# shroglck/open-pi-zero

Measured on AMD Instinct MI355X. Metric: train samples/sec at gbsz 1024 (bf16 fwd+bwd+clip+AdamW), higher is better.
Workload: dtype bf16; 1 GPU; Pi0 bridge training step: 256 img + 20 text + 1 proprio + 4 action tokens; model=pi0 (SigLIP-So400m/14 + Gemma-2B + 0.3B action expert), global_batch=1024, micro_batch=256, grad_accum=4, seq_len=281, parallelism=dp1

## Files before the change

include/pz_abi.h:

```cpp
#ifndef PZ_ABI_H
#define PZ_ABI_H

#include <stdint.h>

#ifdef __cplusplus
extern "C" {
#endif

#define PZ_ABI_VERSION 22

enum {
  PZ_OK = 0,
  PZ_ERR_INVALID_ARG = 1,
  PZ_ERR_LAUNCH = 2,
  PZ_ERR_UNSUPPORTED = 3,
};

enum {
  PZ_EPI_NONE = 0,
  PZ_EPI_GELU = 1,
  PZ_EPI_GEGLU = 2,
  PZ_EPI_SILU = 3,
  PZ_EPI_DGELU = 4,
  PZ_EPI_DSILU = 5,
// ... 47 lines not shown
  float alpha;
  int32_t beta;
} pz_small_gemm_args;
int pz_gemm_small(const pz_small_gemm_args* args, void* stream);

int pz_rmsnorm_fwd(const void* x, int64_t ldx, const void* w, void* y, int64_t ldy, float* rstd,
                   int64_t R, int64_t D, float eps, void* stream);
int pz_rmsnorm_bwd(const void* dy, int64_t lddy, const void* x, int64_t ldx, const void* w,
                   const float* rstd, const void* dres, void* dx, int64_t lddx, float* dw_part,
                   int64_t R, int64_t D, void* stream);
int pz_layernorm_fwd(const void* x, int64_t ldx, const void* w, const void* b, void* y, int64_t ldy,
                     float* mean, float* rstd, int64_t R, int64_t D, float eps, void* stream);
int pz_layernorm_bwd(const void* dy, int64_t lddy, const void* x, int64_t ldx, const void* w,
                     const float* mean, const float* rstd, const void* dres, void* dx, int64_t lddx,
                     float* dw_part, float* db_part, int64_t R, int64_t D, float* dx_part, void* stream);
int64_t pz_norm_rows_per_part(void);
int pz_reduce_parts(const float* part, int64_t P, int64_t D, void* out, int32_t beta, void* stream);
typedef struct pz_reduce_seg {
  const float* part; int64_t P, D; void* out; int32_t beta;
} pz_reduce_seg;
int pz_reduce_parts_multi(const pz_reduce_seg* segs, int32_t nseg, void* stream);
int pz_act_bwd_colsum(const void* dh, int64_t lddh, const void* pre, int64_t ldpre, void* dpre, int64_t M, int64_t N,
                      int32_t act, float* ws, int64_t ws_rows, void* dbias, int32_t beta, void* stream);
int pz_colsum(const void* X, int64_t ld, int64_t M, int64_t N, void* out, int32_t beta, float* ws,
              void* stream);
int pz_batch_sum(const void* X, int64_t B, int64_t stride, int64_t n, void* out, int32_t beta, void* stream);

int pz_rope_table(float* cs, int64_t max_pos, int64_t head_dim, float theta, void* stream);
int pz_qkv_rope_split(const void* qkv, const int64_t* pos, const float* cs, void* q_out, void* k_out,
                      void* v_out, int64_t B, int64_t T, int64_t nh, int64_t nkv, int64_t hd,
                      int64_t Lq, int64_t qoff, int64_t Lk, int64_t koff, void* stream);
typedef struct pz_qkv_rope_args {
  const void* x; int64_t ldx;
  const void* W; int64_t ldw;
  int64_t M, N, K;
  const void* norm_w; float norm_eps;
  const int64_t* pos; const float* cs;
  void* q_out; void* k_out; void* v_out;
  int64_t T, nh, hd, Lq, qoff, Lk, koff;
  int32_t w_fp8; float w_scale;
  const void* x2; int64_t ldx2;
  const void* W2; int64_t ldw2;
  int64_t K2;
} pz_qkv_rope_args;
int pz_gemv_qkv_rope(const pz_qkv_rope_args* a, void* stream);
int pz_gemm_qkv_rope(const pz_qkv_rope_args* a, void* stream);
// ... 186 lines not shown
```

open-pi-zero_amd/csrc/pz_gemm.hip:

```cpp
#include <stdarg.h>
#include <stdio.h>
#include <stdlib.h>
#include <string.h>

#include <type_traits>

#include "pz_gemm_epi.h"

namespace {

constexpr int BM = 128, BN = 128, BK = 64, NT = 256;
constexpr int TILE_BYTES = 128 * 64 * 2;


__device__ __forceinline__ i32x8 cat_f8(const bf16x8& lo, const bf16x8& hi) {
  const u32x4 a = __builtin_bit_cast(u32x4, lo), b = __builtin_bit_cast(u32x4, hi);
  return i32x8{(int)a[0], (int)a[1], (int)a[2], (int)a[3], (int)b[0], (int)b[1], (int)b[2], (int)b[3]};
}

__device__ __forceinline__ int sw_tr(int k) { return ((k & 3) | (((k >> 3) & 1) << 2)) << 2; }

template <bool KC>
__device__ __forceinline__ void g2r(u32x4 (&r)[4], const bf16_t* __restrict__ base, int64_t ld,
                                    int64_t row0, int64_t R, int64_t k0, int64_t K,
// ... 562 lines not shown
          dg[e] = v[e] * x1[e] * gr_;
          du[e] = v[e] * gl_;
        }
        st16(Cp, pack8v(dg));
        st16(Cp + p.geglu_I, pack8v(du));
      } else if (FM == FM_DACT) {
#pragma unroll
        for (int e = 0; e < 8; ++e) v[e] *= gelu ? gelu_tanh_grad(x0[e]) : silu_grad(x0[e]);
        st16(Cp, pack8v(v));
      } else {
        if (act) {
          if (p.aux) st16(p.aux + (m0 + row) * p.ld_aux + n0 + col, iv[i]);
#pragma unroll
          for (int e = 0; e < 8; ++e) v[e] = gelu ? gelu_tanh(v[e]) : silu(v[e]);
        }
#pragma unroll
        for (int e = 0; e < 8; ++e) v[e] += x1[e] + x0[e];
        st16(Cp, pack8v(v));
      }
    }
  }
}

__device__ __forceinline__ void epi8p_rope(const GemmP& p, int64_t m0, int64_t n0, int wr, int wc, int lane,
                                           const f32x4 (&acc)[8][4], char* smem) {
  const int g4 = 4 * (lane >> 4), rl = lane & 15;
  char* img = smem + (wc >> 1) * 65536;
#pragma unroll
  for (int rb = 0; rb < 8; ++rb)
#pragma unroll
    for (int cb = 0; cb < 4; ++cb) {
      float v[4];
#pragma unroll
      for (int r = 0; r < 4; ++r) v[r] = acc[rb][cb][r] * p.alpha;
      img_put(img, wr * 128 + rb * 16 + rl, (wc & 1) * 64 + cb * 16 + g4, u32x2{pack2bf(v[0], v[1]), pack2bf(v[2], v[3])});
    }
  lds_sync();
  const int64_t h = n0 >> 8;
#pragma unroll 2
  for (int it = 0; it < 8; ++it) {
    const int c = threadIdx.x + it * NT2, row = c >> 4, ch = c & 15;
    const int64_t m = m0 + row;
    if (m >= p.M) continue;
    const int off = (ch ^ (row & 15)) << 4;
    const u32x4 w1 = *reinterpret_cast<const u32x4*>(smem + row * 256 + off);
    const u32x4 w2 = *reinterpret_cast<const u32x4*>(smem + 65536 + row * 256 + off);
// ... 2 lines not shown
      bf16_t* dv = p.rv + (b * p.rLk + p.rkoff + t) * 256 + ch * 8;
      *reinterpret_cast<u32x4*>(dv) = w1;
      *reinterpret_cast<u32x4*>(dv + 128) = w2;
      continue;
    }
    float x1[8], x2[8], o1[8], o2[8];
    unpack8(w1, x1);
    unpack8(w2, x2);
    const float4* cs = reinterpret_cast<const float4*>(p.rcs + p.rpos[m] * 256 + 16 * ch);
#pragma unroll
    for (int q = 0; q < 4; ++q) {
      const float4 c2 = cs[q];
      const float co0 = c2.x, si0 = c2.y, co1 = c2.z, si1 = c2.w;
      rope_pair(x1[2 * q], x2[2 * q], co0, si0, o1[2 * q], o2[2 * q]);
      rope_pair(x1[2 * q + 1], x2[2 * q + 1], co1, si1, o1[2 * q + 1], o2[2 * q + 1]);
    }
    bf16_t* d = h < p.rnh ? p.rq + (b * p.rLq + p.rqoff + t) * (p.rnh * 256) + h * 256 + ch * 8
                          : p.rk + (b * p.rLk + p.rkoff + t) * 256 + ch * 8;
    *reinterpret_cast<u32x4*>(d) = pack8v(o1);
    *reinterpret_cast<u32x4*>(d + 128) = pack8v(o2);
  }
}

template <bool GEGLU>
__device__ __forceinline__ void epilogue8p(const GemmP& p, int64_t cofs, int64_t rofs, int64_t m0, int64_t n0,
                                           int wr, int wc, int lane, const f32x4 (&acc)[8][4], char* smem) {
  if (!GEGLU && p.rcs) {
    epi8p_rope(p, m0, n0, wr, wc, lane, acc, smem);
    return;
  }
  const int g4 = 4 * (lane >> 4), rl = lane & 15;
  if (GEGLU) {
    if (m0 + BT <= p.M && n0 + BT / 2 <= p.geglu_I && p.aux) {
#pragma unroll
      for (int rb = 0; rb < 8; ++rb) {
        const int64_t m = m0 + wr * 128 + rb * 16 + rl;
        bf16_t* Ur = p.aux + m * p.ld_aux + p.geglu_I + n0 + wc * 32 + g4;
#pragma unroll
        for (int j = 0; j < 2; ++j) {
          float gg[4], hh[4], uu[4];
#pragma unroll
          for (int r = 0; r < 4; ++r) {
            gg[r] = acc[rb][j][r] * p.alpha;
            uu[r] = acc[rb][2 + j][r] * p.alpha;
            hh[r] = gelu_tanh(gg[r]) * uu[r];
          }
          const int row = wr * 128 + rb * 16 + rl, col = wc * 32 + j * 16 + g4;
          img_put(smem, row, col, u32x2{pack2bf(hh[0], hh[1]), pack2bf(hh[2], hh[3])});
          img_put(smem + 65536, row, col, u32x2{pack2bf(gg[0], gg[1]), pack2bf(gg[2], gg[3])});
// ... 41 lines not shown
        bf16_t* C = reinterpret_cast<bf16_t*>(p.C) + cofs + m0 * p.ldc + n0;
        img_flush(smem, C, p.ldc);
        img_flush(smem + 65536, C + 128, p.ldc);
        break;
      }
      case FM_F32: epi8p_fast<FM_F32>(p, cofs, rofs, m, nb, acc); break;
      case FM_DACT: epi8p_staged<FM_DACT>(p, cofs, rofs, m0, n0, wr, wc, lane, acc, smem); break;
      case FM_DGEGLU: epi8p_staged<FM_DGEGLU>(p, cofs, rofs, m0, n0, wr, wc, lane, acc, smem); break;
      default: epi8p_staged<FM_BF16>(p, cofs, rofs, m0, n0, wr, wc, lane, acc, smem); break;
    }
    return;
  }
  f32x4* park = reinterpret_cast<f32x4*>(smem) + (wr * 4 + wc) * 1024 + lane;
#pragma unroll
  for (int half = 0; half < 2; ++half) {
#pragma unroll
    for (int g = 0; g < 16; ++g) park[g * 64] = acc[half * 4 + (g >> 2)][g & 3];
#pragma unroll 1
    for (int g = 0; g < 16; ++g)
      store_out4_rt(p, cofs, rofs, m + (half * 4 + (g >> 2)) * 16, nb + (g & 3) * 16, park[g * 64]);
  }
}

template <bool AKC, bool BKC, bool GEGLU, bool KTAIL, bool F8, bool EXT = false>
__device__ __forceinline__ void gemm8p_body(const GemmP& p) {
  static_assert(!EXT || (KTAIL && !F8), "rank extension: bf16, tail-capable instantiation");
  static_assert(AKC, "a k-strided A takes gemm8k_kernel (use_khalf)");
  extern __shared__ __attribute__((aligned(16))) char smem[];
  const int nk1 = (int)((p.K + 63) / 64);
  const int nk_all = EXT ? nk1 + (int)((p.K2 + 63) / 64) : nk1;
  int lid = blockIdx.x, piece = -1, kt0 = 0, nk = nk_all;
  if (p.tail_s && lid >= p.dp_tiles) {
    const int u = lid - p.dp_tiles;
    piece = u;
    lid = p.dp_tiles + u / p.tail_s;
    kt0 = (u % p.tail_s) * p.tail_kt;
    nk = min(nk_all - kt0, p.tail_kt);
  }
  int tm, tn;
  tile_coords(lid, p.tiles_m * p.tiles_n, p.tiles_m, p.tiles_n, tm, tn, p.group);
  const int64_t m0 = (int64_t)tm * BT;
  const int64_t n0 = GEGLU ? (int64_t)tn * (BT / 2) : (int64_t)tn * BT;
  const int t = threadIdx.x, lane = t & 63;
  const int wave = __builtin_amdgcn_readfirstlane(t >> 6);
  const int wr = wave >> 2, wc = wave & 3;
  const int64_t z = blockIdx.y;
  const int64_t zo = z / p.batch_inner, zi = z % p.batch_inner;
  const bf16_t* Ab = p.A + zo * p.sAo + zi * p.sAi;
  const bf16_t* Bb = p.B + zo * p.sBo + zi * p.sBi;
// ... 177 lines not shown
    mfma_quad(1, 1);
    mfma_quad(1, 0);
    PZ_RAW_BARRIER();
  }
  if (wr == 0) PZ_RAW_BARRIER();
  if (F8 && p.rs) {
#pragma unroll
    for (int rb = 0; rb < 8; ++rb) {
      const int64_t row = min(m0 + wr * 128 + 16 * rb + (lane & 15), p.M - 1);
      const float sr = p.rs[row];
#pragma unroll
      for (int cb = 0; cb < 4; ++cb) acc[rb][cb] *= sr;
    }
  }

  if (piece >= 0) {
    f32x4* W = reinterpret_cast<f32x4*>(p.ws) + (int64_t)piece * (32 * NT2);
#pragma unroll
    for (int rb = 0; rb < 8; ++rb)
#pragma unroll
      for (int cb = 0; cb < 4; ++cb) W[(rb * 4 + cb) * NT2 + t] = acc[rb][cb];
    return;
  }
  epilogue8p<GEGLU>(p, zo * p.sCo + zi * p.sCi, zo * p.sRo + zi * p.sRi, m0, n0, wr, wc, lane, acc, smem);
}

template <bool AKC, bool BKC, bool GEGLU, bool KTAIL>
__global__ void __launch_bounds__(NT2, 1) gemm8p_kernel(GemmP p) {
  gemm8p_body<AKC, BKC, GEGLU, KTAIL, false>(p);
}

template <bool AKC, bool BKC, bool GEGLU>
__global__ void __launch_bounds__(NT2, 1) gemm8p_x_kernel(GemmP p) {
  gemm8p_body<AKC, BKC, GEGLU, true, false, true>(p);
}

template <bool GEGLU, bool KTAIL>
__global__ void __launch_bounds__(NT2, 1) gemm8p_f8_kernel(GemmP p) {
  gemm8p_body<true, true, GEGLU, KTAIL, true>(p);
}

constexpr int KH_REG = 16384;

template <bool GEGLU>
__device__ __forceinline__ int64_t kh_rowB(int v, int64_t row0, int64_t R, int64_t gI) {
  if (GEGLU) {
    int64_t g = row0 + (v >> 6) * 32 + (v & 31);
    g = g < gI ? g : gI - 1;
    return ((v >> 5) & 1) ? gI + g : g;
  }
  const int64_t g = row0 + v;
  return g < R ? g : R - 1;
// ... 847 lines not shown
  return PZ_OK;
}

template <bool AKC, bool BKC, bool GEGLU>
static int launch8p(const GemmP& p, int64_t batch, hipStream_t st) {
  if (p.K % 64 != 0) return launch8p_k<AKC, BKC, GEGLU, true>(p, batch, st);
  return launch8p_k<AKC, BKC, GEGLU, false>(p, batch, st);
}

template <bool BKC, bool GEGLU>
static int launch8p_x(const GemmP& p, hipStream_t st) {
  const int smem = 2 * P8_BUF;
  auto kern = gemm8p_x_kernel<true, BKC, GEGLU>;
  static bool attr_set = false;
  if (!attr_set) {
    hipFuncSetAttribute((const void*)kern, hipFuncAttributeMaxDynamicSharedMemorySize, smem);
    attr_set = true;
  }
  hipLaunchKernelGGL(kern, dim3(p.tiles_m * p.tiles_n, 1), dim3(NT2), smem, st, p);
  PZ_CHECK_LAUNCH();
  return PZ_OK;
}

extern "C" int pz_gemm(const pz_gemm_args* a, void* stream) {
  PZ_CHECK_ARG(a != nullptr, "pz_gemm: null args");
  PZ_CHECK_ARG(a->M > 0 && a->N > 0 && a->K > 0, "pz_gemm: bad dims M=%lld N=%lld K=%lld",
               (long long)a->M, (long long)a->N, (long long)a->K);
  PZ_CHECK_ARG(a->A && a->B && a->C, "pz_gemm: null operand");
  PZ_CHECK_ARG(a->batch >= 1 && a->batch_inner >= 1 && a->batch % a->batch_inner == 0,
               "pz_gemm: bad batch %lld/%lld", (long long)a->batch, (long long)a->batch_inner);
  PZ_CHECK_ARG(PZ_ALIGNED(a->A, 16) && PZ_ALIGNED(a->B, 16), "pz_gemm: A/B must be 16-byte aligned");
  PZ_CHECK_ARG(a->lda % 8 == 0 && a->ldb % 8 == 0, "pz_gemm: lda/ldb must be multiples of 8");
  PZ_CHECK_ARG(a->ldc % 4 == 0 && PZ_ALIGNED(a->C, 8), "pz_gemm: ldc %% 4 and C 8-byte alignment");
  PZ_CHECK_ARG(a->sA_outer % 8 == 0 && a->sA_inner % 8 == 0 && a->sB_outer % 8 == 0 &&
                   a->sB_inner % 8 == 0 && a->sC_outer % 4 == 0 && a->sC_inner % 4 == 0,
               "pz_gemm: batch strides must keep 16-byte alignment");
  if (a->a_kcontig) PZ_CHECK_ARG(a->K % 8 == 0, "pz_gemm: k-contiguous A needs K %% 8 == 0");
  else PZ_CHECK_ARG(a->M % 8 == 0, "pz_gemm: k-strided A needs M %% 8 == 0");
  if (a->b_kcontig) PZ_CHECK_ARG(a->K % 8 == 0, "pz_gemm: k-contiguous B needs K %% 8 == 0");
  else PZ_CHECK_ARG(a->N % 8 == 0, "pz_gemm: k-strided B needs N %% 8 == 0");
  const bool geglu = a->epilogue == PZ_EPI_GEGLU;
  if (geglu) {
    PZ_CHECK_ARG(a->b_kcontig && a->geglu_inter > 0 && a->N == 2 * a->geglu_inter && a->batch == 1 &&
                     !a->beta_accum && !a->resid && !a->bias && !a->c_fp32 && a->geglu_inter % 4 == 0,
                 "pz_gemm: GEGLU needs k-contiguous B = [gate; up] (N = 2I), no batch/bias/resid");
  }
  if (a->epilogue == PZ_EPI_GELU || a->epilogue == PZ_EPI_SILU)
// ... 61 lines not shown
  p.sBo = a->sB_outer; p.sBi = a->sB_inner;
  p.sCo = a->sC_outer; p.sCi = a->sC_inner;
  p.sRo = a->sR_outer; p.sRi = a->sR_inner;
  p.epi = a->epilogue;
  p.c_fp32 = a->c_fp32;
  p.beta = a->beta_accum;
  p.alpha = a->alpha;
  p.nw = (const bf16_t*)a->norm_w;
  p.neps = a->norm_eps;
  p.rs = a->fp8_mode == 1 ? a->a_row_scale : nullptr;
  if (a->K2 > 0) {
    p.A2 = (const bf16_t*)a->A2;
    p.B2 = (const bf16_t*)a->B2;
    p.lda2 = a->lda2; p.ldb2 = a->ldb2; p.K2 = a->K2;
  }
  hipStream_t st = (hipStream_t)stream;

  const Plan pl = make_plan(a);
  {
    const char* e = getenv("PZ_GEMM_GROUP");
    if (e && atoi(e) >= 1 && atoi(e) <= 64) p.group = atoi(e);
    else p.group = (a->K >= 16384 && pl.tiles_n <= 8) || a->epilogue == PZ_EPI_DGEGLU ? 2 : 8;
  }
  if (pl.kind == PATH_GEMV) return pz_gemv_launch(a, st);
  if (a->norm_w)
    PZ_CHECK_ARG((pl.kind == PATH_SKINNY || pl.kind == PATH_SKINNY64) && PZ_ALIGNED(a->norm_w, 16),
                 "pz_gemm: fused RMSNorm needs the few-row paths (M <= 64, k-contiguous A/B, K %% 32 == 0 "
                 "(M <= 16) or K %% 64 == 0) and a 16-byte aligned weight");
  if (pl.kind == PATH_SKINNY64) {
    p.tiles_n = (int)pl.tiles_n;
    if (pl.ksplit > 0) {
      p.ws = (float*)a->workspace;
      p.ksplit = pl.ksplit;
      p.ldw = pl.ldw;
      p.sk_tk = sk64_fits(pl, a) ? 0 : -1;
    }
    return pz_sk64_launch(p, pl.skinny_w, pl.skinny_mb, a->fp8_mode == 2, pl.tiles_n, st);
  }
  if (a->fp8_mode == 1 && pl.kind == PATH_ROWS) {
    p.tiles_m = (int)pl.tiles_m;
    p.tiles_n = (int)pl.tiles_n;
    PZ_CHECK_ARG(PZ_ALIGNED(a->A, 16) && PZ_ALIGNED(a->B, 16), "pz_gemm: W8A8 rows need 16-byte aligned codes");
    return pz_rows_launch(p, pl.rows_w, pl.rows_tnb, false, 2, st);
  }
  if (a->fp8_mode == 1) {
    p.tiles_m = (int)pl.tiles_m;
// ... 47 lines not shown
    if (geglu) {
      if (a->a_kcontig) return launch8p<true, true, true>(p, a->batch, st);
      return launch8p<false, true, true>(p, a->batch, st);
    }
    if (a->a_kcontig && a->b_kcontig) return launch8p<true, true, false>(p, a->batch, st);
    if (a->a_kcontig && !a->b_kcontig) return launch8p<true, false, false>(p, a->batch, st);
    if (!a->a_kcontig && a->b_kcontig) return launch8p<false, true, false>(p, a->batch, st);
    return launch8p<false, false, false>(p, a->batch, st);
  }
  if (pl.kind == PATH_SPLIT) {
    p.ws = (float*)a->workspace;
    p.ksplit = pl.ksplit;
    p.ldw = pl.ldw;
  }
  if (geglu) {
    if (pl.tag) return launch_tile_any<true, true, 4, 1>(p, pl, a->batch, st);
    if (a->a_kcontig) return launch_tile_any<true, true, 4, 0>(p, pl, a->batch, st);
    return launch_tile_any<false, true, 4, 0>(p, pl, a->batch, st);
  }
  if (a->a_kcontig && a->b_kcontig) return launch_tile_any<true, true, 2, 0>(p, pl, a->batch, st);
  if (a->a_kcontig && !a->b_kcontig) return launch_tile_any<true, false, 2, 0>(p, pl, a->batch, st);
  if (!a->a_kcontig && a->b_kcontig) return launch_tile_any<false, true, 2, 0>(p, pl, a->batch, st);
  return launch_tile_any<false, false, 2, 0>(p, pl, a->batch, st);
}

extern "C" int pz_gemm_qkv_rope(const pz_qkv_rope_args* a, void* stream) {
  PZ_CHECK_ARG(a && a->x && a->W && a->pos && a->cs && a->k_out && a->v_out && a->M > 0 && a->K > 0,
               "gemm_qkv_rope: bad args");
  PZ_CHECK_ARG(a->nh >= 1 && a->N == (a->nh + 2) * a->hd && a->T > 0 && a->M % a->T == 0,
               "gemm_qkv_rope: N = (nh + 2) * hd, M %% T == 0");
  if (a->hd != BT || !a->q_out) return PZ_ERR_UNSUPPORTED;
  PZ_CHECK_ARG(PZ_ALIGNED(a->x, 16) && PZ_ALIGNED(a->W, 16) && a->ldx % 8 == 0 && a->ldw % 8 == 0 && a->K % 8 == 0 &&
                   PZ_ALIGNED(a->q_out, 16) && PZ_ALIGNED(a->k_out, 16) && PZ_ALIGNED(a->v_out, 16),
               "gemm_qkv_rope: 16-byte alignment");
  pz_gemm_args g;
  memset(&g, 0, sizeof(g));
  g.M = a->M; g.N = a->N; g.K = a->K;
  g.A = a->x; g.lda = a->ldx; g.a_kcontig = 1;
  g.B = a->W; g.ldb = a->ldw; g.b_kcontig = 1;
  g.C = a->q_out; g.ldc = a->N;
  g.batch = 1; g.batch_inner = 1;
  g.alpha = 1.f;
  g.norm_w = a->norm_w;
  g.norm_eps = a->norm_eps;
  if (a->K2 > 0) {
    if (a->w_fp8 || a->norm_w) return PZ_ERR_UNSUPPORTED;
// ... 79 lines not shown
```

open-pi-zero_amd/csrc/pz_gemm_epi.h:

```cpp
#pragma once

#include <type_traits>

#include "pz_common.h"

struct GemmP {
  const bf16_t* A;
  const bf16_t* B;
  void* C;
  const bf16_t* bias;
  const bf16_t* resid;
  bf16_t* aux;
  int64_t M, N, K, lda, ldb, ldc, ld_resid, ld_aux, geglu_I;
  int64_t batch_inner, sAo, sAi, sBo, sBi, sCo, sCi, sRo, sRi;
  int tiles_m, tiles_n, epi, c_fp32, beta;
  float alpha;
  float* ws;
  int64_t ksplit, ldw;
  int sk_tk;
  int batch_xcd;
  int dp_tiles, tail_s, tail_kt;
  const bf16_t* nw;
  float neps;
  const float* rs;
  const int64_t* rpos;
  const float* rcs;
  bf16_t *rq, *rk, *rv;
  int64_t rT, rnh, rLq, rqoff, rLk, rkoff;
  int group;
  const bf16_t* A2;
  const bf16_t* B2;
  int64_t lda2, ldb2, K2;
};

namespace {

__device__ __forceinline__ void tile_coords(int bid, int nwg, int tiles_m, int tiles_n, int& tm, int& tn,
                                            int GROUP = 8) {
  const int xcd = bid & 7, local = bid >> 3;
  const int q = nwg >> 3, r = nwg & 7;
  const int wg = (xcd < r ? xcd * (q + 1) : r * (q + 1) + (xcd - r) * q) + local;
  GROUP = GROUP >= 1 ? GROUP : 8;
  const int per_group = GROUP * tiles_n;
  const int g = wg / per_group;
  const int first_m = g * GROUP;
  const int gsize = min(tiles_m - first_m, GROUP);
  const int in = wg - g * per_group;
  tm = first_m + in % gsize;
  tn = in / gsize;
}

struct Side {
  u32x4 w;
};

// ... 258 lines not shown
```

open-pi-zero_amd/pizero_native/_lib.py:

```python

from __future__ import annotations

import ctypes as C
import os

_HERE = os.path.dirname(os.path.dirname(os.path.abspath(__file__)))
LIB_PATH = os.path.join(_HERE, "libpizero_hip.so")
if os.environ.get("PZ_LIB_PATH"):
    LIB_PATH = os.path.join(_HERE, os.path.basename(os.environ["PZ_LIB_PATH"]))
    import sys as _sys

    print(f"[pizero_native] PZ_LIB_PATH override: loading {LIB_PATH} instead of the default libpizero_hip.so",
          file=_sys.stderr, flush=True)

ABI_VERSION = 22
PZ_EPI_NONE, PZ_EPI_GELU, PZ_EPI_GEGLU, PZ_EPI_SILU = 0, 1, 2, 3
PZ_EPI_DGELU, PZ_EPI_DSILU, PZ_EPI_DGEGLU = 4, 5, 6
PZ_SUMSQ_PARTS = 2048
PZ_OBS_MAX_TAPS, PZ_OBS_MAX_EXTENT = 64, 16384
PZ_OBS_NORM_BOUND, PZ_OBS_NORM_GAUSSIAN = 0, 1
PZ_AUG_CROP, PZ_AUG_BRIGHTNESS, PZ_AUG_CONTRAST, PZ_AUG_SATURATION, PZ_AUG_HUE, PZ_AUG_ALL = 1, 2, 4, 8, 16, 31

i64, i32, f32, vp = C.c_int64, C.c_int32, C.c_float, C.c_void_p
fp = C.POINTER(C.c_float)
# ... 88 lines not shown
        ("v_bstride", i64), ("o", vp), ("ldo", i64), ("B", i64), ("nh", i64), ("T", i64), ("nk", i64),
        ("head_dim", i64), ("scale", f32), ("cap", f32), ("cnt", vp), ("prefix", i64), ("cond", i64),
        ("qtok0", i64), ("ws", vp), ("ws_bytes", i64),
    ]


SIGNATURES = {
    "pz_gemm": [C.POINTER(GemmArgs), vp],
    "pz_fp8_quant_rows": [vp, i64, vp, i64, vp, i64, i64, vp],
    "pz_fp8_quant_tensor": [vp, i64, vp, f32, vp],
    "pz_fp8_quant_vt": [vp, i64, i64, i64, i64, vp, vp, i64, vp],
    "pz_rmsnorm_fwd_f8": [vp, i64, vp, vp, i64, vp, i64, i64, f32, vp],
    "pz_layernorm_fwd_f8": [vp, i64, vp, vp, vp, i64, vp, i64, i64, f32, vp],
    "pz_fp8_quant_attn": [vp, i64, vp, i64, vp, i64, i64, i64, i64, vp, vp, vp, vp, vp, vp, i64, vp],
    "pz_flash_fwd_f8": [C.POINTER(FlashArgs), vp, vp, vp, vp, i64, vp, vp, i64, vp],
    "pz_fp8_absmax": [vp, i64, vp, vp],
    "pz_gemm_kernel_name": [C.POINTER(GemmArgs)],
    "pz_gemm_small": [C.POINTER(SmallGemmArgs), vp],
    "pz_rmsnorm_fwd": [vp, i64, vp, vp, i64, vp, i64, i64, f32, vp],
    "pz_rmsnorm_bwd": [vp, i64, vp, i64, vp, vp, vp, vp, i64, vp, i64, i64, vp],
    "pz_layernorm_fwd": [vp, i64, vp, vp, vp, i64, vp, vp, i64, i64, f32, vp],
    "pz_layernorm_bwd": [vp, i64, vp, i64, vp, vp, vp, vp, vp, i64, vp, vp, i64, i64, vp, vp],
    "pz_act_bwd_colsum": [vp, i64, vp, i64, vp, i64, i64, i32, vp, i64, vp, i32, vp],
    "pz_reduce_parts_multi": [vp, i32, vp],
    "pz_norm_rows_per_part": [],
    "pz_reduce_parts": [vp, i64, i64, vp, i32, vp],
    "pz_colsum": [vp, i64, i64, i64, vp, i32, vp, vp],
    "pz_batch_sum": [vp, i64, i64, i64, vp, i32, vp],
    "pz_rope_table": [vp, i64, i64, f32, vp],
    "pz_qkv_rope_split": [vp, vp, vp, vp, vp, vp, i64, i64, i64, i64, i64, i64, i64, i64, i64, vp],
    "pz_qkv_rope_split_bwd": [vp, vp, vp, vp, vp, vp, i64, i64, i64, i64, i64, i64, i64, i64, i64, vp],
    "pz_gemv_qkv_rope": [C.POINTER(QkvRopeArgs), vp],
    "pz_gemm_qkv_rope": [C.POINTER(QkvRopeArgs), vp],
    "pz_decode_attn": [C.POINTER(DecodeAttnArgs), vp],
    "pz_decode_attn_ws_bytes": [i64, i64, i64],
    "pz_attn_softmax": [C.POINTER(SoftmaxArgs), vp],
    "pz_attn_softmax_bwd": [vp, vp, i64, vp, vp, i64, i64, i64, f32, f32, vp],
    "pz_flash_fwd": [C.POINTER(FlashArgs), vp],
    "pz_flash_fwd_probs": [C.POINTER(FlashArgs), vp, vp, i64, vp],
    "pz_flash_bwd_ds": [C.POINTER(FlashArgs), vp, vp, vp, i64, vp],
    "pz_flash_bwd_prep": [C.POINTER(FlashArgs), vp],
    "pz_flash_bwd": [C.POINTER(FlashArgs), vp],
    "pz_patchify": [vp, vp, i64, i64, i64, i64, i64, vp],
    "pz_embed_merge": [vp, vp, i64, vp, vp, i64, i64, i64, i64, i64, i64, f32, f32, vp],
    "pz_embed_merge_bwd": [vp, vp, vp, i64, i64, i64, i64, i64, f32, vp],
    "pz_time_embed": [vp, vp, i64, i64, f32, i32, vp],
# ... 47 lines not shown
class NativeError(RuntimeError):
    pass


def lib():
    global _lib
    if _lib is None:
        if not os.path.exists(LIB_PATH):
            raise NativeError(
                f"{LIB_PATH} not found: build it with `python open-pi-zero_amd/build_native.py` "
                "(or __graft_entry__.build()); the Pi0 path has no CPU/eager fallback")
        L = C.CDLL(LIB_PATH)
        for name, argt in SIGNATURES.items():
            fn = getattr(L, name)
            fn.argtypes = argt
            fn.restype = _RESTYPE.get(name, C.c_int)
        if L.pz_abi_version() != ABI_VERSION:
            raise NativeError(f"{LIB_PATH}: ABI version {L.pz_abi_version()} != {ABI_VERSION}; rebuild it")
        _lib = L
    return _lib


_NO_LAUNCH = {"pz_last_error", "pz_abi_version", "pz_gemm_kernel_name", "pz_norm_rows_per_part",
              "pz_decode_attn_ws_bytes", "pz_lora_wgrad_ws_bytes", "pz_debug_poison_lds",
              "pz_image_resize_scratch_bytes", "pz_image_augment_scratch_bytes"}
_POISON_LDS = [0xFFFFFFFF if os.environ.get("PZ_POISON_LDS", "0") == "1" else None]


_RECENT = [[] if os.environ.get("PZ_CHECK_FINITE", "0") == "1" else None]


def recent_launches(clear=True):
    r = _RECENT[0] or []
    if clear and _RECENT[0] is not None:
        _RECENT[0] = []
    return r


def set_poison_lds(word):
    _POISON_LDS[0] = None if word is None else int(word) & 0xFFFFFFFF


def call(name, *args):
    if _POISON_LDS[0] is not None and name not in _NO_LAUNCH:
        rc = lib().pz_debug_poison_lds(_POISON_LDS[0], args[-1])
        if rc != 0:
# ... 9 lines not shown
```

open-pi-zero_amd/pizero_native/engine.py:

```python

from __future__ import annotations

import contextlib
import functools
import math
import os
import weakref
from dataclasses import dataclass

import torch

from . import ops
from .ops import PZ_EPI_DGEGLU, PZ_EPI_GEGLU, PZ_EPI_GELU, PZ_EPI_NONE, PZ_EPI_SILU

BF16 = torch.bfloat16
F32 = torch.float32


def _cfg(cfg, key, default=None):
    from src.utils.config import cfg_get

    return cfg_get(cfg, key, default)


# ... 242 lines not shown

    return wrap


class Group:

    def __init__(self, name, prefix, T, joint_off, hidden, inter, theta, skip_last):
        self.name, self.prefix = name, prefix
        self.T, self.off, self.hid, self.inter, self.theta = T, joint_off, hidden, inter, theta
        self.skip_last = skip_last


class Engine:
    def __init__(self, model):
        self.m = model
        self.d = Dims.from_cfg(model.cfg)
        self._tables = {}
        self._ws = {}
        self._jkv_holder = None
        self.joint_flash = False
        self.joint_probs = True
        self.infer_flash = True
        self.fuse_qkv_rope = self.d.hd == 256
        self.expert_stream = True
        self.expert_stream_fwd = False
        self.sig_pitch = (self.d.vI + 63) // 64 * 64
        self._side = {}
        self.check_finite = os.environ.get("PZ_CHECK_FINITE", "0") == "1"
        self.f8 = None
        self.f8_version = None
        self._lora_sites = {}
        self._lora_w = frozenset(n[: -len("lora_A")] + "weight" for n in self.ar.slots if n.endswith(".lora_A"))
        self._merged = None
        self._merged_ver = None
        self._infer = False
        if self.d.nkv != 1:
            raise NotImplementedError("joint attention kernel path assumes MQA (num_key_value_heads=1, bridge.yaml:176)")

    def ada_slots(self, prefix):
        key = ("ada_slots", prefix)
        sl = self._tables.get(key)
        if sl is None:
            from src.model.vla.pizero import adaln_slots

            sl = self._tables[key] = adaln_slots(prefix, self.d.nL, self.d.ada)
        return sl
# ... 13 lines not shown
    def span(self, first, last):
        return self.ar.span(first, last, self._merged if self._infer and first in self._lora_w else None)

    def lora(self, *wnames):
        if wnames[0] not in self._lora_w:
            return None
        st = self._lora_sites.get(wnames)
        if st is None:
            st = self._lora_sites[wnames] = LoraSite(self, wnames)
        return st

    def _linear(self, x, names, W, out, train, fp8=True, gemm=ops.linear, **kw):
        if not train:
            if fp8:
                self.lin(x, names[0], W, out, **kw)
            else:
                ops.linear(x, W, out, **kw)
            return None
        site = self.lora(*names)
        lo = site.fwd(x) if site is not None else None
        gemm(x, W, out, lora=lo, **kw)
        return lo[0] if lo else None

    def _dgrad(self, names, x, u, dy, W, dx, beta, wgrad=None, **kw):
        site = self.lora(*names)
        lo = None
        if site is not None:
            lo = site.bwd(dy)
            site.grads(x, u, dy, lo[0], beta)
        if wgrad is not None:
            wgrad()
        ops.linear_dgrad(dy, W, dx, lora=lo, **kw)

    def lora_refresh(self):
        if not self._lora_w:
            return False
        ver = self.weights_version()
        if self._merged is not None and self._merged_ver == ver and self._merged.device == self.ar.data.device:
            return False
        from src.model.lora import LORA_SCALING

        if self._merged is None or self._merged.device != self.ar.data.device:
            self._merged = torch.empty_like(self.ar.data)
        for wn in sorted(self._lora_w):
            W = self.ar.view(wn)
            A = self.ar.view(wn[: -len("weight")] + "lora_A")
            Bm = self.ar.view(wn[: -len("weight")] + "lora_B")
            out, inn = W.shape
            ops.gemm(out, inn, A.shape[0], Bm, A.shape[0], True, A, inn, False, self.ar.view(wn, self._merged), inn,
                     alpha=LORA_SCALING, resid=W, ld_resid=inn)
        self._merged_ver = ver
        return True

    def gw(self, name):
        return self.ar.grad_view(name)
# ... 252 lines not shown
            ops.linear_wgrad(dimg, sv["y"], self.gw(nm + "weight"), beta=beta)
        if self.rg(nm + "bias"):
            ops.colsum(dimg, self.gw(nm + "bias"), ws, beta=beta)
        dy = torch.empty(M, d.vH, device=dev, dtype=BF16)
        self._dgrad([nm + "weight"], sv["y"], sv["u_proj"], dimg, self.w(nm + "weight"), dy, beta)
        dx = torch.empty_like(dy)
        ops.layernorm_bwd(dy, sv["x_last"], self.w(vt + "post_layernorm.weight"), sv["mu"], sv["r"], dx,
                          dw_part=pw, db_part=pb, dx_part=pd)
        self._norm_grads(vt + "post_layernorm.", pw, pb, beta)
        nh, hd = d.vheads, d.vH // d.vheads
        Np = d.img_tok
        W3 = 3 * d.vH
        dg = self._sig_rows(M, dev)
        delta = torch.empty(B * nh, Np, device=dev, dtype=F32)
        dqkv = torch.empty(M, W3, device=dev, dtype=BF16)
        dh = torch.empty(M, d.vH, device=dev, dtype=BF16)
        dxm = torch.empty(M, d.vH, device=dev, dtype=BF16)
        dO = torch.empty(M, d.vH, device=dev, dtype=BF16)
        for i in reversed(range(d.vL)):
            p = f"{vt}encoder.layers.{i}."
            st = sv["layers"][i]
            red = []
            fc1b = self.rg(p + "mlp.fc1.bias")
            self._dgrad([p + "mlp.fc2.weight"], st["g1"], st["u_fc2"], dx, self.w(p + "mlp.fc2.weight"), dg, beta)
            if fb and fc1b:
                ops.act_bwd_colsum(dg, st["a1"], dg, PZ_EPI_GELU, ws_act, self.gw(p + "mlp.fc1.bias"), beta=beta)
            else:
                ops.act_bwd(dg, st["a1"], dg, None, PZ_EPI_GELU)
            if self.rg(p + "mlp.fc2.weight"):
                ops.linear_wgrad(dx, st["g1"], self.gw(p + "mlp.fc2.weight"), beta=beta)
            st["g1"] = None
            if self.rg(p + "mlp.fc2.bias"):
                if fb:
                    self._reduce(red, pd, self.gw(p + "mlp.fc2.bias"), beta)
                else:
                    ops.colsum(dx, self.gw(p + "mlp.fc2.bias"), ws, beta=beta)
            if self.rg(p + "mlp.fc1.weight"):
                ops.linear_wgrad(dg, st["h2"], self.gw(p + "mlp.fc1.weight"), beta=beta)
            if fc1b and not fb:
                ops.colsum(dg, self.gw(p + "mlp.fc1.bias"), ws, beta=beta)
            self._dgrad([p + "mlp.fc1.weight"], st["h2"], st["u_fc1"], dg, self.w(p + "mlp.fc1.weight"), dh, beta)
            ops.layernorm_bwd(dh, st["xm"], self.w(p + "layer_norm2.weight"), st["mu2"], st["r2"], dxm, dres=dx,
                              dw_part=pw2, db_part=pb2, dx_part=pd2)
            self._norm_grads(p + "layer_norm2.", pw2, pb2, beta, red)
            if self.rg(p + "self_attn.out_proj.weight"):
                ops.linear_wgrad(dxm, st["O"], self.gw(p + "self_attn.out_proj.weight"), beta=beta)
            if self.rg(p + "self_attn.out_proj.bias"):
                if fb:
                    self._reduce(red, pd2, self.gw(p + "self_attn.out_proj.bias"), beta)
                else:
                    ops.colsum(dxm, self.gw(p + "self_attn.out_proj.bias"), ws, beta=beta)
# ... 970 lines not shown
```

open-pi-zero_amd/pizero_native/ops.py:

```python

from __future__ import annotations

import ctypes as C

import torch

from ._lib import (
    PZ_EPI_DGEGLU,
    PZ_EPI_DGELU,
    PZ_EPI_DSILU,
    PZ_EPI_GEGLU,
    PZ_EPI_GELU,
    PZ_EPI_NONE,
    PZ_EPI_SILU,
    PZ_OBS_MAX_EXTENT,
    PZ_OBS_MAX_TAPS,
    PZ_OBS_NORM_BOUND,
    PZ_OBS_NORM_GAUSSIAN,
    PZ_SUMSQ_PARTS,
    AdamW8Args,
    QkvRopeArgs,
    DecodeAttnArgs,
    FlashArgs,
    GemmArgs,
# ... 299 lines not shown
         mod.stride(0), R, D, int(rows_per_sample), float(eps), _st())


def adaln_norm_bwd(dh, x, rstd, mod, gamma, dx, dmod, beta, rows_per_sample, dres=None):
    R, D = x.shape
    call("pz_adaln_norm_bwd", _p(dh), dh.stride(0), _p(x), x.stride(0), _p(rstd), mod[:, gamma[0]:].data_ptr(),
         _p(gamma[1]), _p(dres), _p(dx), dx.stride(0), None if dmod is None else dmod[:, gamma[0]:].data_ptr(),
         None if dmod is None else dmod[:, beta:].data_ptr(), mod.stride(0), R, D, int(rows_per_sample), _st())
    return dx


def adaln_gate_bwd(dout, y, mod, gate, dy, dmod, rows_per_sample):
    R, D = y.shape
    call("pz_adaln_gate_bwd", _p(dout), dout.stride(0), _p(y), y.stride(0), mod[:, gate[0]:].data_ptr(), _p(gate[1]),
         _p(dy), dy.stride(0), dmod[:, gate[0]:].data_ptr(), mod.stride(0), R, D, int(rows_per_sample), _st())
    return dy


def act_bwd_colsum(dh, pre, dpre, act, ws, dbias, beta=False):
    M, N = pre.shape
    call("pz_act_bwd_colsum", _p(dh), dh.stride(0), _p(pre), pre.stride(0), _p(dpre), M, N, int(act), _p(ws),
         ws.numel() // N, _p(dbias), int(beta), _st())
    return dpre


_RPP = None


def rows_per_part():
    global _RPP
    if _RPP is None:
        from ._lib import lib

        _RPP = int(lib().pz_norm_rows_per_part())
    return _RPP


def reduce_parts(part, out, beta=False):
    P, D = part.shape
    call("pz_reduce_parts", _p(part), P, D, _p(out), int(beta), _st())
    return out


def reduce_parts_multi(items, beta=False):
    from ._lib import ReduceSeg

# ... 540 lines not shown
```

Before: 276.4 samples/s.

## Fuse GELU-backward and fc1 bias column sums into the fc2 dgrad GEMM epilogue

```diff
diff --git a/include/pz_abi.h b/include/pz_abi.h
--- a/include/pz_abi.h
+++ b/include/pz_abi.h
@@ -93,6 +93,9 @@
 int pz_reduce_parts_multi(const pz_reduce_seg* segs, int32_t nseg, void* stream);
 int pz_act_bwd_colsum(const void* dh, int64_t lddh, const void* pre, int64_t ldpre, void* dpre, int64_t M, int64_t N,
                       int32_t act, float* ws, int64_t ws_rows, void* dbias, int32_t beta, void* stream);
+int pz_gemm_dact_colsum_fits(const pz_gemm_args* args, int64_t ws_rows);
+int pz_gemm_dact_colsum(const pz_gemm_args* args, float* ws, int64_t ws_rows, void* dbias, int32_t beta,
+                        void* stream);
 int pz_colsum(const void* X, int64_t ld, int64_t M, int64_t N, void* out, int32_t beta, float* ws,
               void* stream);
 int pz_batch_sum(const void* X, int64_t B, int64_t stride, int64_t n, void* out, int32_t beta, void* stream);
diff --git a/open-pi-zero_amd/csrc/pz_gemm.hip b/open-pi-zero_amd/csrc/pz_gemm.hip
--- a/open-pi-zero_amd/csrc/pz_gemm.hip
+++ b/open-pi-zero_amd/csrc/pz_gemm.hip
@@ -608,6 +608,73 @@
   }
 }
 
+__device__ __forceinline__ void epi8p_dact_cs(const GemmP& p, int64_t m0, int64_t n0, int wr, int wc, int lane,
+                                              const f32x4 (&acc)[8][4], char* smem) {
+  const int g4 = 4 * (lane >> 4), rl = lane & 15;
+  char* img = smem + (wc >> 1) * 65536;
+#pragma unroll
+  for (int cb = 0; cb < 4; ++cb)
+#pragma unroll
+    for (int rb = 0; rb < 8; ++rb) {
+      float v[4];
+#pragma unroll
+      for (int r = 0; r < 4; ++r) v[r] = acc[rb][cb][r] * p.alpha;
+      img_put(img, wr * 128 + rb * 16 + rl, (wc & 1) * 64 + cb * 16 + g4, u32x2{pack2bf(v[0], v[1]), pack2bf(v[2], v[3])});
+    }
+  lds_sync();
+  const int rows = (int)(p.M - m0 < BT ? p.M - m0 : BT), cols = (int)(p.N - n0 < BT ? p.N - n0 : BT);
+  bf16_t* C = reinterpret_cast<bf16_t*>(p.C) + m0 * p.ldc + n0;
+  const bf16_t* X = p.aux + m0 * p.ld_aux + n0;
+  const bool gelu = p.epi == PZ_EPI_DGELU;
+  constexpr int CPB = 4;
+#pragma unroll
+  for (int half = 0; half < 16 / CPB; ++half) {
+    u32x4 a0[CPB], iv[CPB];
+#pragma unroll
+    for (int i = 0; i < CPB; ++i) {
+      const int c = threadIdx.x + (half * CPB + i) * NT2;
+      const int im = c >> 12, row = (c >> 4) & 255, ch = c & 15;
+      const int col = im * 128 + ch * 8;
+      iv[i] = *reinterpret_cast<const u32x4*>(smem + im * 65536 + row * 256 + ((ch ^ (row & 15)) << 4));
+      a0[i] = row < rows && col < cols ? *reinterpret_cast<const u32x4*>(X + row * p.ld_aux + col)
+                                       : u32x4{0u, 0u, 0u, 0u};
+    }
+#pragma unroll
+    for (int i = 0; i < CPB; ++i) {
+      const int c = threadIdx.x + (half * CPB + i) * NT2;
+      const int im = c >> 12, row = (c >> 4) & 255, ch = c & 15;
+      const int col = im * 128 + ch * 8;
+      const bool ok = row < rows && col < cols;
+      float v[8], x0[8];
+      unpack8(iv[i], v);
+      unpack8(a0[i], x0);
+#pragma unroll
+      for (int e = 0; e < 8; ++e) v[e] *= gelu ? gelu_tanh_grad(x0[e]) : silu_grad(x0[e]);
+      const u32x4 o = ok ? pack8v(v) : u32x4{0u, 0u, 0u, 0u};
+      if (ok) st16(C + row * p.ldc + col, o);
+      *reinterpret_cast<u32x4*>(smem + im * 65536 + row * 256 + ((ch ^ (row & 15)) << 4)) = o;
+    }
+  }
+  lds_sync();
+  const int rpc = p.cs_rpc;
+  const int items = 128 * (BT / rpc);
+  for (int it = threadIdx.x; it < items; it += NT2) {
+    const int col = 2 * (it & 127), r0 = (it >> 7) * rpc;
+    if (r0 >= rows || col >= cols) continue;
+    const int ch = (col & 127) >> 3;
+    const char* src = smem + (col >> 7) * 65536 + (col & 7) * 2;
+    float s0 = 0.f, s1 = 0.f;
+#pragma unroll 8
+    for (int r = r0; r < r0 + rpc; ++r) {
+      const unsigned w = *reinterpret_cast<const unsigned*>(src + r * 256 + ((ch ^ (r & 15)) << 4));
+      s0 += __uint_as_float(w << 16);
+      s1 += __uint_as_float(w & 0xffff0000u);
+    }
+    *reinterpret_cast<u32x2*>(p.cs + ((m0 + r0) / rpc) * p.cs_ld + n0 + col) =
+        u32x2{__float_as_uint(s0), __float_as_uint(s1)};
+  }
+}
+
 __device__ __forceinline__ void epi8p_rope(const GemmP& p, int64_t m0, int64_t n0, int wr, int wc, int lane,
                                            const f32x4 (&acc)[8][4], char* smem) {
   const int g4 = 4 * (lane >> 4), rl = lane & 15;
@@ -656,9 +723,13 @@
   }
 }
 
-template <bool GEGLU>
+template <bool GEGLU, bool CS = false>
 __device__ __forceinline__ void epilogue8p(const GemmP& p, int64_t cofs, int64_t rofs, int64_t m0, int64_t n0,
                                            int wr, int wc, int lane, const f32x4 (&acc)[8][4], char* smem) {
+  if constexpr (CS) {
+    epi8p_dact_cs(p, m0, n0, wr, wc, lane, acc, smem);
+    return;
+  }
   if (!GEGLU && p.rcs) {
     epi8p_rope(p, m0, n0, wr, wc, lane, acc, smem);
     return;
@@ -746,9 +817,10 @@
   }
 }
 
-template <bool AKC, bool BKC, bool GEGLU, bool KTAIL, bool F8, bool EXT = false>
+template <bool AKC, bool BKC, bool GEGLU, bool KTAIL, bool F8, bool EXT = false, bool CS = false>
 __device__ __forceinline__ void gemm8p_body(const GemmP& p) {
   static_assert(!EXT || (KTAIL && !F8), "rank extension: bf16, tail-capable instantiation");
+  static_assert(!CS || (!GEGLU && !F8), "column partial sums: the plain bf16 DGELU / DSILU dgrad");
   static_assert(AKC, "a k-strided A takes gemm8k_kernel (use_khalf)");
   extern __shared__ __attribute__((aligned(16))) char smem[];
   const int nk1 = (int)((p.K + 63) / 64);
@@ -972,12 +1044,17 @@
       for (int cb = 0; cb < 4; ++cb) W[(rb * 4 + cb) * NT2 + t] = acc[rb][cb];
     return;
   }
-  epilogue8p<GEGLU>(p, zo * p.sCo + zi * p.sCi, zo * p.sRo + zi * p.sRi, m0, n0, wr, wc, lane, acc, smem);
+  epilogue8p<GEGLU, CS>(p, zo * p.sCo + zi * p.sCi, zo * p.sRo + zi * p.sRi, m0, n0, wr, wc, lane, acc, smem);
 }
 
 template <bool AKC, bool BKC, bool GEGLU, bool KTAIL>
 __global__ void __launch_bounds__(NT2, 1) gemm8p_kernel(GemmP p) {
   gemm8p_body<AKC, BKC, GEGLU, KTAIL, false>(p);
+}
+
+template <bool EXT>
+__global__ void __launch_bounds__(NT2, 1) gemm8p_cs_kernel(GemmP p) {
+  gemm8p_body<true, false, false, EXT, false, EXT, true>(p);
 }
 
 template <bool AKC, bool BKC, bool GEGLU>
@@ -1871,7 +1948,44 @@
   return PZ_OK;
 }
 
-extern "C" int pz_gemm(const pz_gemm_args* a, void* stream) {
+template <bool EXT>
+static int launch8p_cs(const GemmP& p, hipStream_t st) {
+  const int smem = 2 * P8_BUF;
+  auto kern = gemm8p_cs_kernel<EXT>;
+  static bool attr_set = false;
+  if (!attr_set) {
+    hipFuncSetAttribute((const void*)kern, hipFuncAttributeMaxDynamicSharedMemorySize, smem);
+    attr_set = true;
+  }
+  hipLaunchKernelGGL(kern, dim3(p.tiles_m * p.tiles_n, 1), dim3(NT2), smem, st, p);
+  PZ_CHECK_LAUNCH();
+  return PZ_OK;
+}
+
+static bool dact_cs_fits(const pz_gemm_args* a, const Plan& pl, int64_t ws_rows, int64_t* rpc) {
+  if (a->epilogue != PZ_EPI_DGELU && a->epilogue != PZ_EPI_DSILU) return false;
+  if (pl.kind != PATH_256 || pl.tail_s || pl.geglu || !pl.akc || pl.bkc || a->batch != 1 || a->fp8_mode != 0 ||
+      a->c_fp32 || a->norm_w || ws_rows <= 0)
+    return false;
+  if (a->K2 == 0 && (a->K % 64 != 0 || use_khalf(true, false, a->M, a->N, a->K))) return false;
+  if (a->N % 8 != 0 || a->ldc % 8 != 0 || a->ld_aux % 8 != 0 || !PZ_ALIGNED(a->C, 16) || !PZ_ALIGNED(a->aux, 16))
+    return false;
+  int64_t chunks = ws_rows < (a->M + 15) / 16 ? ws_rows : (a->M + 15) / 16;
+  const int64_t r = (a->M + chunks - 1) / chunks;
+  if (r < 16 || BT % r != 0 || a->M % r != 0) return false;
+  *rpc = r;
+  return true;
+}
+
+namespace {
+struct DactCs {
+  float* ws;
+  int64_t ws_rows;
+  int64_t rpc;
+};
+}
+
+static int gemm_run(const pz_gemm_args* a, void* stream, DactCs* cs) {
   PZ_CHECK_ARG(a != nullptr, "pz_gemm: null args");
   PZ_CHECK_ARG(a->M > 0 && a->N > 0 && a->K > 0, "pz_gemm: bad dims M=%lld N=%lld K=%lld",
                (long long)a->M, (long long)a->N, (long long)a->K);
@@ -1979,6 +2093,18 @@
     if (e && atoi(e) >= 1 && atoi(e) <= 64) p.group = atoi(e);
     else p.group = (a->K >= 16384 && pl.tiles_n <= 8) || a->epilogue == PZ_EPI_DGEGLU ? 2 : 8;
   }
+  if (cs) {
+    int64_t rpc = 0;
+    if (!dact_cs_fits(a, pl, cs->ws_rows, &rpc)) return PZ_ERR_UNSUPPORTED;
+    PZ_CHECK_ARG(pl.tiles_m * pl.tiles_n < (1LL << 31), "pz_gemm_dact_colsum: grid too large");
+    p.tiles_m = (int)pl.tiles_m;
+    p.tiles_n = (int)pl.tiles_n;
+    p.cs = cs->ws;
+    p.cs_ld = a->N;
+    p.cs_rpc = (int)rpc;
+    cs->rpc = rpc;
+    return a->K2 > 0 ? launch8p_cs<true>(p, st) : launch8p_cs<false>(p, st);
+  }
   if (pl.kind == PATH_GEMV) return pz_gemv_launch(a, st);
   if (a->norm_w)
     PZ_CHECK_ARG((pl.kind == PATH_SKINNY || pl.kind == PATH_SKINNY64) && PZ_ALIGNED(a->norm_w, 16),
@@ -2072,6 +2198,25 @@
   if (a->a_kcontig && !a->b_kcontig) return launch_tile_any<true, false, 2, 0>(p, pl, a->batch, st);
   if (!a->a_kcontig && a->b_kcontig) return launch_tile_any<false, true, 2, 0>(p, pl, a->batch, st);
   return launch_tile_any<false, false, 2, 0>(p, pl, a->batch, st);
+}
+
+extern "C" int pz_gemm(const pz_gemm_args* a, void* stream) { return gemm_run(a, stream, nullptr); }
+
+extern "C" int pz_gemm_dact_colsum_fits(const pz_gemm_args* a, int64_t ws_rows) {
+  if (!a || a->M <= 0 || a->N <= 0 || a->K <= 0 || !a->C || !a->aux) return 0;
+  int64_t rpc = 0;
+  return dact_cs_fits(a, make_plan(a), ws_rows, &rpc) ? 1 : 0;
+}
+
+extern "C" int pz_gemm_dact_colsum(const pz_gemm_args* a, float* ws, int64_t ws_rows, void* dbias, int32_t beta,
+                                   void* stream) {
+  PZ_CHECK_ARG(a && ws && PZ_ALIGNED(ws, 16) && ws_rows > 0, "pz_gemm_dact_colsum: bad args");
+  PZ_CHECK_ARG(a->epilogue == PZ_EPI_DGELU || a->epilogue == PZ_EPI_DSILU,
+               "pz_gemm_dact_colsum: a PZ_EPI_DGELU / PZ_EPI_DSILU dgrad only");
+  DactCs cs{ws, ws_rows, 0};
+  const int rc = gemm_run(a, stream, &cs);
+  if (rc != PZ_OK || !dbias) return rc;
+  return pz_reduce_parts(ws, a->M / cs.rpc, a->N, dbias, beta, stream);
 }
 
 extern "C" int pz_gemm_qkv_rope(const pz_qkv_rope_args* a, void* stream) {
diff --git a/open-pi-zero_amd/csrc/pz_gemm_epi.h b/open-pi-zero_amd/csrc/pz_gemm_epi.h
--- a/open-pi-zero_amd/csrc/pz_gemm_epi.h
+++ b/open-pi-zero_amd/csrc/pz_gemm_epi.h
@@ -31,6 +31,9 @@
   const bf16_t* A2;
   const bf16_t* B2;
   int64_t lda2, ldb2, K2;
+  float* cs;
+  int64_t cs_ld;
+  int cs_rpc;
 };
 
 namespace {
diff --git a/open-pi-zero_amd/pizero_native/_lib.py b/open-pi-zero_amd/pizero_native/_lib.py
--- a/open-pi-zero_amd/pizero_native/_lib.py
+++ b/open-pi-zero_amd/pizero_native/_lib.py
@@ -134,6 +134,8 @@
     "pz_layernorm_fwd": [vp, i64, vp, vp, vp, i64, vp, vp, i64, i64, f32, vp],
     "pz_layernorm_bwd": [vp, i64, vp, i64, vp, vp, vp, vp, vp, i64, vp, vp, i64, i64, vp, vp],
     "pz_act_bwd_colsum": [vp, i64, vp, i64, vp, i64, i64, i32, vp, i64, vp, i32, vp],
+    "pz_gemm_dact_colsum_fits": [C.POINTER(GemmArgs), i64],
+    "pz_gemm_dact_colsum": [C.POINTER(GemmArgs), vp, i64, vp, i32, vp],
     "pz_reduce_parts_multi": [vp, i32, vp],
     "pz_norm_rows_per_part": [],
     "pz_reduce_parts": [vp, i64, i64, vp, i32, vp],
@@ -227,6 +229,7 @@
 
 
 _NO_LAUNCH = {"pz_last_error", "pz_abi_version", "pz_gemm_kernel_name", "pz_norm_rows_per_part",
+              "pz_gemm_dact_colsum_fits",
               "pz_decode_attn_ws_bytes", "pz_lora_wgrad_ws_bytes", "pz_debug_poison_lds",
               "pz_image_resize_scratch_bytes", "pz_image_augment_scratch_bytes"}
 _POISON_LDS = [0xFFFFFFFF if os.environ.get("PZ_POISON_LDS", "0") == "1" else None]
diff --git a/open-pi-zero_amd/pizero_native/engine.py b/open-pi-zero_amd/pizero_native/engine.py
--- a/open-pi-zero_amd/pizero_native/engine.py
+++ b/open-pi-zero_amd/pizero_native/engine.py
@@ -288,6 +288,7 @@
         self.joint_probs = True
         self.infer_flash = True
         self.fuse_qkv_rope = self.d.hd == 256
+        self.fuse_dact_colsum = True
         self.expert_stream = True
         self.expert_stream_fwd = False
         self.sig_pitch = (self.d.vI + 63) // 64 * 64
@@ -347,7 +348,7 @@
         gemm(x, W, out, lora=lo, **kw)
         return lo[0] if lo else None
 
-    def _dgrad(self, names, x, u, dy, W, dx, beta, wgrad=None, **kw):
+    def _dgrad(self, names, x, u, dy, W, dx, beta, wgrad=None, gemm=ops.linear_dgrad, **kw):
         site = self.lora(*names)
         lo = None
         if site is not None:
@@ -355,7 +356,7 @@
             site.grads(x, u, dy, lo[0], beta)
         if wgrad is not None:
             wgrad()
-        ops.linear_dgrad(dy, W, dx, lora=lo, **kw)
+        gemm(dy, W, dx, lora=lo, **kw)
 
     def lora_refresh(self):
         if not self._lora_w:
@@ -654,11 +655,17 @@
             st = sv["layers"][i]
             red = []
             fc1b = self.rg(p + "mlp.fc1.bias")
-            self._dgrad([p + "mlp.fc2.weight"], st["g1"], st["u_fc2"], dx, self.w(p + "mlp.fc2.weight"), dg, beta)
-            if fb and fc1b:
-                ops.act_bwd_colsum(dg, st["a1"], dg, PZ_EPI_GELU, ws_act, self.gw(p + "mlp.fc1.bias"), beta=beta)
+            if fb and fc1b and self.fuse_dact_colsum:
+                self._dgrad([p + "mlp.fc2.weight"], st["g1"], st["u_fc2"], dx, self.w(p + "mlp.fc2.weight"), dg, beta,
+                            gemm=lambda dy, W, out, lora=None: ops.dgrad_act_colsum(
+                                dy, W, out, st["a1"], PZ_EPI_GELU, ws_act, self.gw(p + "mlp.fc1.bias"), beta=beta,
+                                lora=lora, red=red))
             else:
-                ops.act_bwd(dg, st["a1"], dg, None, PZ_EPI_GELU)
+                self._dgrad([p + "mlp.fc2.weight"], st["g1"], st["u_fc2"], dx, self.w(p + "mlp.fc2.weight"), dg, beta)
+                if fb and fc1b:
+                    ops.act_bwd_colsum(dg, st["a1"], dg, PZ_EPI_GELU, ws_act, self.gw(p + "mlp.fc1.bias"), beta=beta)
+                else:
+                    ops.act_bwd(dg, st["a1"], dg, None, PZ_EPI_GELU)
             if self.rg(p + "mlp.fc2.weight"):
                 ops.linear_wgrad(dx, st["g1"], self.gw(p + "mlp.fc2.weight"), beta=beta)
             st["g1"] = None
diff --git a/open-pi-zero_amd/pizero_native/ops.py b/open-pi-zero_amd/pizero_native/ops.py
--- a/open-pi-zero_amd/pizero_native/ops.py
+++ b/open-pi-zero_amd/pizero_native/ops.py
@@ -345,6 +345,51 @@
     call("pz_act_bwd_colsum", _p(dh), dh.stride(0), _p(pre), pre.stride(0), _p(dpre), M, N, int(act), _p(ws),
          ws.numel() // N, _p(dbias), int(beta), _st())
     return dpre
+
+
+def _dact_args(dy, W, dx, pre, act, lora):
+    M, N = dy.shape
+    K = W.shape[1]
+    epi = PZ_EPI_DGELU if act == PZ_EPI_GELU else PZ_EPI_DSILU
+    a = _args(M, K, N, dy, dy.stride(0), True, W, W.stride(0), False, dx, dx.stride(0), epi, 1.0, False, None, None, 0,
+              pre, pre.stride(0), 0, 1, 1, (0, 0), (0, 0), (0, 0), (0, 0), workspace(dx.device))
+    if lora is not None:
+        a.A2, a.lda2, a.B2, a.ldb2, a.K2 = _p(lora[0]), lora[0].stride(0), _p(lora[1]), lora[1].stride(0), \
+            lora[0].shape[1]
+    return a
+
+
+def dgrad_act_colsum_fits(dy, W, dx, pre, act, ws, lora=None):
+    a = _dact_args(dy, W, dx, pre, act, lora)
+    return bool(lib().pz_gemm_dact_colsum_fits(C.byref(a), ws.numel() // W.shape[1]))
+
+
+def dgrad_act_colsum(dy, W, dx, pre, act, ws, dbias, beta=False, lora=None, red=None, fused=True):
+    K = W.shape[1]
+    ws_rows = ws.numel() // K
+    if fused:
+        a = _dact_args(dy, W, dx, pre, act, lora)
+        if lib().pz_gemm_dact_colsum_fits(C.byref(a), ws_rows):
+            probe = _PROBE is not None and _PROBE[0](a.M, a.N, a.K, a.epilogue, 1)
+            if probe:
+                e0, e1 = torch.cuda.Event(enable_timing=True), torch.cuda.Event(enable_timing=True)
+                e0.record()
+            call("pz_gemm_dact_colsum", C.byref(a), _p(ws), ws_rows, None if red is not None else _p(dbias),
+                 int(bool(beta)), _st())
+            if probe:
+                e1.record()
+                _PROBE[1].append((e0, e1))
+            if red is not None:
+                M = dy.shape[0]
+                chunks = min(ws_rows, (M + 15) // 16)
+                chunks = M // ((M + chunks - 1) // chunks)
+                red.append((ws.view(-1)[: chunks * K].view(chunks, K), dbias))
+            return True
+    if dx.stride(0) != pre.stride(0):
+        raise ValueError("dgrad_act_colsum: dx and pre need one row pitch (pz_act_bwd_colsum writes dpre at pre's)")
+    linear_dgrad(dy, W, dx, lora=lora)
+    act_bwd_colsum(dx, pre, dx, act, ws, dbias, beta=beta)
+    return False
 
 
 _RPP = None
```

Result: no change. 277.8 samples/s (median of 6 runs) (+0.5%).
